# kritsanan1/Qwen3-TTS

Measured on AMD Instinct MI355X. Metric: audio-seconds/sec (RTF) + p50 first-packet latency, 1.7B @ batch 1/8, 1->8 GPU, higher is better.
Workload: dtype bf16; 1 GPU; Qwen3-TTS-12Hz-1.7b-customvoice B=8/GPU x 200-token prompts, streaming text, 256 frames + codec decode; global_batch=8, seq_len=200, frames=256, parallelism=dp1

## Files before the change

### include/qwen3tts_amd.h

```cpp
#ifndef QWEN3TTS_AMD_H
#define QWEN3TTS_AMD_H

#ifdef __cplusplus
extern "C" {
#endif

enum { QT_F32 = 0, QT_BF16 = 1 };
enum { QT_ACT_NONE = 0, QT_ACT_SILU = 1, QT_ACT_GELU = 2, QT_ACT_RELU = 3, QT_ACT_SIGMOID = 4,
       QT_ACT_RELU_TANH = 5  };
enum { QT_AACT_NONE = 0, QT_AACT_ELU = 1 };
enum { QT_PAD_ZERO = 0, QT_PAD_REFLECT = 1, QT_PAD_REPLICATE = 2 };
enum { QT_EPI_STORE = 0, QT_EPI_ADD = 1, QT_EPI_SWIGLU = 2 };
enum { QT_OK = 0, QT_ERR_ARG = -1, QT_ERR_SHAPE = -2, QT_ERR_DTYPE = -3, QT_ERR_LAUNCH = -4 };

const char* qt_build_id(void);

typedef struct qt_gemm_args {
  int M, N, K;
  int a_dtype, w_dtype, o_dtype;
  const void* A;
  long long lda;
  const int* a_index;
  const void* W;
  const float* gamma;
// ... 38 lines not shown
  const float* cos_tab; const float* sin_tab;
  const int* rope_pos; const int* row_batch; const int* kv_pos;
  float* q_out;
  void* k_cache; void* v_cache; int kv_dtype; int Lmax;
} qt_qkv_args;
int qt_qkv_post(const qt_qkv_args* args, void* stream);

typedef struct qt_attn_args {
  int R, Hq, Hkv, D, Lmax, window;
  const float* q;
  const void* k_cache; const void* v_cache; int kv_dtype;
  const int* row_batch; const int* row_start; const int* row_len;
  void* out; int o_dtype;
  int max_keys;
} qt_attn_args;
int qt_attention(const qt_attn_args* args, void* stream);

typedef struct qt_decode_attn_args {
  int R, Hq, Hkv, D, Lmax, window;
  const float* qkv;
  const float* q_norm; const float* k_norm; float eps;
  const float* cos_tab; const float* sin_tab;
  const int* rope_pos; const int* row_batch; const int* kv_pos; const int* row_start;
  void* k_cache; void* v_cache; int kv_dtype;
  void* out; int o_dtype;
  int const_pos;
  int nsplit;
  void* ws; long long ws_bytes;
} qt_decode_attn_args;
long long qt_decode_attn_ws_bytes(int R, int Hq, int Hkv, int D, int nsplit);
int qt_decode_attention(const qt_decode_attn_args* args, void* stream);
int qt_small_prefill_attention(const qt_decode_attn_args* args, int T, void* stream);

typedef struct qt_attn_oproj_args {
  int R, Hq, Hkv, D, Lmax;
  const float* qkv;
  const float* q_norm; const float* k_norm; float eps;
  const float* cos_tab; const float* sin_tab;
  const int* rope_pos; const int* kv_pos; const int* row_start; int const_pos;
  void* k_cache; void* v_cache; int kv_dtype;
  const void* w_o; int w_dtype; int N;
  float* x; long long ldx;
  void* x16; long long ldx16;
  void* ws; long long ws_bytes;
} qt_attn_oproj_args;
int qt_decode_attn_oproj(const qt_attn_oproj_args* args, void* stream);
long long qt_attn_oproj_ws_bytes(int N, int Hkv);
typedef struct qt_cp_step_args {
  int R, n_layers, Lmax, const_pos, V;
  float eps;
  const float* cos_tab; const float* sin_tab;
  const void* w_qkv[8]; const void* w_o[8]; const void* w_gu[8]; const void* w_down[8];
  const float* q_norm[8]; const float* k_norm[8];
  void* k_cache[8]; void* v_cache[8];
  const void* w_lm;
  const float* x; long long ldx;
  const float* qkv0; long long ldq;
  float* logits; long long ldl;
  void* ws; long long ws_bytes;
} qt_cp_step_args;
int qt_cp_step(const qt_cp_step_args* args, void* stream);
int qt_cp_prefill(const qt_cp_step_args* args, void* stream);
long long qt_cp_step_ws_bytes(void);
long long qt_cp_step_dbg_bytes(void);
int qt_cp_step_supported(int H, int I, int Hq, int Hkv, int D, int n_layers, int V);

int qt_attn_oproj_resident_blocks(void);

typedef struct qt_talker_tail_args {
  int R; float eps;
  const void* att; long long lda;
  float* x; long long ldx;
  const void* w_o; const void* w_gu; const void* w_down;
  const void* w_qkv_next;
  float* qkv; long long ldq;
  void* ws; long long ws_bytes;
  int H, I;
} qt_talker_tail_args;
int qt_talker_tail(const qt_talker_tail_args* args, void* stream);
long long qt_talker_tail_ws_bytes(void);
long long qt_talker_tail_stamp_bytes(void);
long long qt_talker_tail_dbg_bytes(void);
int qt_talker_tail_supported(int H, int I, int Hq, int D, int qkv_w);

typedef struct qt_sample_row {
  float temperature; float top_p; float rep_penalty; int top_k;
  int do_sample; int reserved; unsigned long long seed;
} qt_sample_row;

typedef struct qt_sample_args {
  const float* logits; int R; int V; long long ld;
  unsigned char* seen; float rep_penalty;
  const int* n_generated; int min_new_tokens; int eos_id;
  int suppress_lo, suppress_hi, suppress_keep; int ignore_eos;
  unsigned char* finished;
  int do_sample; int top_k; float top_p; float temperature;
  unsigned long long seed; const int* step; int substep;
  int* tok_out;
  int* codes; long long codes_ld; int codes_w; int codes_col; int codes_step_off;
  int row_base;
  const float* emb_table; int emb_dim; float* emb_out; long long emb_ld;
  const unsigned long long* seed_ptr;
  float debug_u;
  void* emb_out16; long long emb_ld16;
  const float* emb2_table; int emb2_dim; float* emb2_out; long long emb2_ld;
  int algo;
  int ctr_stride;
  const int* philox_row;
  const int* force; int* pick;
  const qt_sample_row* rows;
} qt_sample_args;
int qt_sample(const qt_sample_args* args, void* stream);
long long qt_sample_row_bytes(void);
long long qt_sample_args_bytes(void);
int qt_cp_step_sampled(const qt_cp_step_args* args, const qt_sample_args* sample, void* stream);

int qt_rmsnorm(const float* x, const float* gamma, float eps, float* out, int M, int N, void* stream);
int qt_rmsnorm_rec(const float* x, const float* gamma, float eps, float* out, int M, int N, float* rec,
                   long long rec_ld, const int* step, int step_off, int step_stride, void* stream);

int qt_gather_rows(const void* table, int dtype, const int* idx, int M, int H, float* out, long long ldo, void* stream);

int qt_frame_embed(const void* emb0, const void* emb_cp, int dtype, int V0, int Vcp, int G, int H,
                   const int* codes, long long codes_ld, const int* step, int step_stride, const float* trailing,
                   int T, const float* pad, float* x, void* x16, int B, void* stream);

int qt_advance(int* counters, int n, void* stream);
int qt_advance_rows(int* counters, int B, int nfields, int cap, void* stream);

int qt_trail_append(const float* rows, const int* slots, float* trailing, int B, int T, int H, int n, void* stream);

int qt_stream_window(void* hist, const void* x, void* xin, int dtype, int B, int H, int n, int C,
                     int rows_per_frame, int head, const int* rows, void* stream);
int qt_stream_rows(int* nf, const int* rows, int B, int n, int* pos, int* row_len, void* stream);

int qt_rvq_gather(const float* tables, int Q, int n_first, int cb_size, int dim, const int* codes, int B, int T,
                  float* out_first, float* out_rest, void* stream);
int qt_snake(const void* x, void* y, int dtype, long long rows, int C, const float* alpha, const float* inv_beta,
             void* stream);
int qt_dwconv_ln(const void* x, int dtype, int B, int T, int C, const float* w, const float* b, const float* ln_w,
                 const float* ln_b, float eps, void* out, void* stream);
int qt_clamp_pcm(const void* x, int dtype, long long n, float* out, void* stream);

enum { QT_PCM_F32 = 0, QT_PCM_S16 = 1 };
typedef struct qt_resample_row {
  const float* src;
  void* out;
  const float* hist_in;
  float* hist_out;
  long long pos;
  long long m0;
  int n, count, flush, reserved;
} qt_resample_row;
typedef struct qt_resample_args {
  int up, down, half, taps, H, format, B, reserved;
  const float* table;
  const qt_resample_row* rows;
} qt_resample_args;
int qt_resample(const qt_resample_args* a, void* stream);

int qt_pad_time(const void* x, long long ldx, const void* x2, long long ldx2, int dtype, int B, int T, int C, int left,
                int right, int mode, int t_total, void* out, long long ldo, void* stream);
int qt_zero_tail(void* x, int dtype, int B, int Tp, int v, int C, long long ldx, void* stream);
int qt_layernorm(const float* x, long long ldx, const float* w, const float* b, float eps, void* out, int o_dtype,
                 long long ldo, int M, int N, void* stream);
long long qt_rvq_encode_ws_bytes(int R, int D, int cb);
// ... 16 lines not shown
```

### qwen3-tts_amd/qwen_tts/_hip.py

```python
from __future__ import annotations

import ctypes
import os

import torch

HERE = os.path.dirname(os.path.abspath(__file__))
LIB_PATH = os.environ.get("QWEN3TTS_AMD_LIB",
                          os.path.join(os.path.dirname(HERE), "lib", "libqwen3tts_amd.so"))

F32, BF16 = 0, 1
ACT_NONE, ACT_SILU, ACT_GELU, ACT_RELU, ACT_SIGMOID, ACT_RELU_TANH = 0, 1, 2, 3, 4, 5
AACT_NONE, AACT_ELU = 0, 1
PAD_ZERO, PAD_REFLECT, PAD_REPLICATE = 0, 1, 2
EPI_STORE, EPI_ADD, EPI_SWIGLU = 0, 1, 2
ERRORS = {-1: "bad argument", -2: "bad shape", -3: "unsupported dtype", -4: "launch failed"}

c_int, c_ll, c_float, c_void_p, c_ull = ctypes.c_int, ctypes.c_longlong, ctypes.c_float, ctypes.c_void_p, ctypes.c_ulonglong


class GemmArgs(ctypes.Structure):
    _fields_ = [("M", c_int), ("N", c_int), ("K", c_int), ("a_dtype", c_int), ("w_dtype", c_int), ("o_dtype", c_int),
                ("A", c_void_p), ("lda", c_ll), ("a_index", c_void_p), ("W", c_void_p), ("gamma", c_void_p),
                ("eps", c_float), ("rmsnorm", c_int), ("bias", c_void_p), ("colscale", c_void_p), ("act", c_int), ("epi", c_int),
                ("out", c_void_p), ("ldo", c_ll), ("taps", c_int), ("dil", c_int), ("cin", c_int),
                ("cin_pad", c_int), ("t_in", c_int), ("t_out", c_int), ("t_off", c_int),
                ("ws", c_void_p), ("ws_bytes", c_ll), ("splitk", c_int),
                ("snake_alpha", c_void_p), ("snake_inv_beta", c_void_p), ("a_act", c_int),
                ("out2", c_void_p), ("ldo2", c_ll)]

GEMM_WS_MIN = 4 << 20

(ROUTE_NONE, ROUTE_IM2COL, ROUTE_GEMV, ROUTE_SK, ROUTE_CONV_N1, ROUTE_WT_1x8, ROUTE_WT_2x8, ROUTE_WT_4x4, ROUTE_PF2,
 ROUTE_PF, ROUTE_IGEMM) = range(11)
ROUTE_NAMES = ["NONE", "IM2COL", "GEMV", "SK", "CONV_N1", "WT_1x8", "WT_2x8", "WT_4x4", "PF2", "PF", "IGEMM"]


class GemmRouteInfo(ctypes.Structure):
    _fields_ = [(n, c_int) for n in ("route", "inner", "ks", "mr", "wpb", "u", "fold", "nt_loads", "pf2_cfg", "pf2_ks",
                                     "ntb", "mi", "sk_mi", "ws_split")]


class QkvArgs(ctypes.Structure):
    _fields_ = [("R", c_int), ("Hq", c_int), ("Hkv", c_int), ("D", c_int), ("qkv", c_void_p), ("q_norm", c_void_p),
                ("k_norm", c_void_p), ("eps", c_float), ("cos_tab", c_void_p), ("sin_tab", c_void_p),
                ("rope_pos", c_void_p), ("row_batch", c_void_p), ("kv_pos", c_void_p), ("q_out", c_void_p),
                ("k_cache", c_void_p), ("v_cache", c_void_p), ("kv_dtype", c_int), ("Lmax", c_int)]


class AttnArgs(ctypes.Structure):
    _fields_ = [("R", c_int), ("Hq", c_int), ("Hkv", c_int), ("D", c_int), ("Lmax", c_int), ("window", c_int),
                ("q", c_void_p), ("k_cache", c_void_p), ("v_cache", c_void_p), ("kv_dtype", c_int),
                ("row_batch", c_void_p), ("row_start", c_void_p), ("row_len", c_void_p), ("out", c_void_p),
                ("o_dtype", c_int), ("max_keys", c_int)]


class DecodeAttnArgs(ctypes.Structure):
    _fields_ = [("R", c_int), ("Hq", c_int), ("Hkv", c_int), ("D", c_int), ("Lmax", c_int), ("window", c_int),
                ("qkv", c_void_p), ("q_norm", c_void_p), ("k_norm", c_void_p), ("eps", c_float),
                ("cos_tab", c_void_p), ("sin_tab", c_void_p), ("rope_pos", c_void_p), ("row_batch", c_void_p),
                ("kv_pos", c_void_p), ("row_start", c_void_p), ("k_cache", c_void_p), ("v_cache", c_void_p),
                ("kv_dtype", c_int), ("out", c_void_p), ("o_dtype", c_int), ("const_pos", c_int), ("nsplit", c_int),
                ("ws", c_void_p), ("ws_bytes", c_ll)]


class AttnOprojArgs(ctypes.Structure):
    _fields_ = [("R", c_int), ("Hq", c_int), ("Hkv", c_int), ("D", c_int), ("Lmax", c_int), ("qkv", c_void_p),
                ("q_norm", c_void_p), ("k_norm", c_void_p), ("eps", c_float), ("cos_tab", c_void_p), ("sin_tab", c_void_p),
                ("rope_pos", c_void_p), ("kv_pos", c_void_p), ("row_start", c_void_p), ("const_pos", c_int),
                ("k_cache", c_void_p), ("v_cache", c_void_p), ("kv_dtype", c_int), ("w_o", c_void_p), ("w_dtype", c_int),
                ("N", c_int), ("x", c_void_p), ("ldx", c_ll), ("x16", c_void_p), ("ldx16", c_ll), ("ws", c_void_p),
                ("ws_bytes", c_ll)]


P8 = c_void_p * 8


class CpStepArgs(ctypes.Structure):
    _fields_ = [("R", c_int), ("n_layers", c_int), ("Lmax", c_int), ("const_pos", c_int), ("V", c_int),
                ("eps", c_float), ("cos_tab", c_void_p), ("sin_tab", c_void_p),
                ("w_qkv", P8), ("w_o", P8), ("w_gu", P8), ("w_down", P8), ("q_norm", P8), ("k_norm", P8),
                ("k_cache", P8), ("v_cache", P8), ("w_lm", c_void_p), ("x", c_void_p), ("ldx", c_ll),
                ("qkv0", c_void_p), ("ldq", c_ll), ("logits", c_void_p), ("ldl", c_ll), ("ws", c_void_p),
                ("ws_bytes", c_ll)]


class TalkerTailArgs(ctypes.Structure):
    _fields_ = [("R", c_int), ("eps", ctypes.c_float), ("att", c_void_p), ("lda", c_ll), ("x", c_void_p), ("ldx", c_ll),
                ("w_o", c_void_p), ("w_gu", c_void_p), ("w_down", c_void_p), ("w_qkv_next", c_void_p),
                ("qkv", c_void_p), ("ldq", c_ll), ("ws", c_void_p), ("ws_bytes", c_ll), ("H", c_int), ("I", c_int)]


class SampleRow(ctypes.Structure):
    _fields_ = [("temperature", c_float), ("top_p", c_float), ("rep_penalty", c_float), ("top_k", c_int),
                ("do_sample", c_int), ("reserved", c_int), ("seed", c_ull)]


class SampleArgs(ctypes.Structure):
    _fields_ = [("logits", c_void_p), ("R", c_int), ("V", c_int), ("ld", c_ll), ("seen", c_void_p),
                ("rep_penalty", c_float), ("n_generated", c_void_p), ("min_new_tokens", c_int), ("eos_id", c_int),
                ("suppress_lo", c_int), ("suppress_hi", c_int), ("suppress_keep", c_int), ("ignore_eos", c_int),
                ("finished", c_void_p), ("do_sample", c_int), ("top_k", c_int), ("top_p", c_float),
                ("temperature", c_float), ("seed", c_ull), ("step", c_void_p), ("substep", c_int),
                ("tok_out", c_void_p), ("codes", c_void_p), ("codes_ld", c_ll), ("codes_w", c_int),
                ("codes_col", c_int), ("codes_step_off", c_int), ("row_base", c_int),
                ("emb_table", c_void_p), ("emb_dim", c_int), ("emb_out", c_void_p), ("emb_ld", c_ll),
                ("seed_ptr", c_void_p), ("debug_u", c_float), ("emb_out16", c_void_p), ("emb_ld16", c_ll),
                ("emb2_table", c_void_p), ("emb2_dim", c_int), ("emb2_out", c_void_p), ("emb2_ld", c_ll),
                ("algo", c_int), ("ctr_stride", c_int), ("philox_row", c_void_p), ("force", c_void_p),
                ("pick", c_void_p), ("rows", c_void_p)]


PCM_F32, PCM_S16 = 0, 1


class ResampleRow(ctypes.Structure):
    _fields_ = [("src", c_void_p), ("out", c_void_p), ("hist_in", c_void_p), ("hist_out", c_void_p), ("pos", c_ll),
                ("m0", c_ll), ("n", c_int), ("count", c_int), ("flush", c_int), ("reserved", c_int)]


class ResampleArgs(ctypes.Structure):
    _fields_ = [("up", c_int), ("down", c_int), ("half", c_int), ("taps", c_int), ("H", c_int), ("format", c_int),
                ("B", c_int), ("reserved", c_int), ("table", c_void_p), ("rows", ctypes.POINTER(ResampleRow))]


EXPORTS = ["qt_gemm", "qt_gemm_route", "qt_tile_weight", "qt_qkv_post", "qt_attention", "qt_decode_attention", "qt_decode_attn_ws_bytes",
           "qt_rmsnorm_rec", "qt_small_prefill_attention",
           "qt_decode_attn_oproj", "qt_attn_oproj_ws_bytes", "qt_attn_oproj_resident_blocks",
           "qt_cp_step", "qt_cp_prefill", "qt_cp_step_sampled", "qt_cp_step_ws_bytes", "qt_cp_step_supported", "qt_cp_step_dbg_bytes",
           "qt_talker_tail", "qt_talker_tail_ws_bytes", "qt_talker_tail_stamp_bytes", "qt_talker_tail_dbg_bytes",
           "qt_talker_tail_supported",
           "qt_sample", "qt_sample_row_bytes", "qt_sample_args_bytes", "qt_rmsnorm", "qt_gather_rows", "qt_frame_embed", "qt_advance", "qt_advance_rows",
           "qt_stream_window", "qt_stream_rows", "qt_trail_append",
           "qt_rvq_gather", "qt_snake", "qt_dwconv_ln", "qt_clamp_pcm", "qt_resample",
           "qt_pad_time", "qt_zero_tail", "qt_layernorm", "qt_rvq_encode", "qt_rvq_encode_ws_bytes", "qt_mel_logmag", "qt_time_stats",
           "qt_scale_add", "qt_bcast_rows", "qt_build_id"]

_LIB = None
BUILD_ID = None


def source_digest(probe=False):
    bpath = os.path.join(os.path.dirname(HERE), "build.py")
    if not os.path.exists(bpath) or not os.path.isdir(os.path.join(os.path.dirname(HERE), "csrc")):
        return None
    import importlib.util
    spec = importlib.util.spec_from_file_location("_qt_build", bpath)
    mod = importlib.util.module_from_spec(spec)
    spec.loader.exec_module(mod)
    return mod.source_digest(probe=probe) + ("-probe" if probe else "")


def load_library(path: str = LIB_PATH):
    if not os.path.exists(path):
        raise RuntimeError(f"HIP library not found at {path}: run `python qwen3-tts_amd/build.py` "
                           "(or __graft_entry__.build()); there is no CPU fallback")
    L = ctypes.CDLL(path)
    L.qt_build_id.restype = ctypes.c_char_p
    L.qt_build_id.argtypes = []
    bid = L.qt_build_id().decode()
    want = source_digest(probe=os.path.basename(path).endswith("_probe.so")) if path == LIB_PATH else None
    if want is not None and bid != want and os.environ.get("QT_ALLOW_STALE_LIB") != "1":
        raise RuntimeError(f"{path} was built from other sources (build id {bid}, sources {want}): rebuild with "
                           "`python qwen3-tts_amd/build.py`")
    global BUILD_ID
    BUILD_ID = bid
    P = c_void_p
    sig = {
        "qt_gemm": [P, P], "qt_gemm_route": [P, P], "qt_tile_weight": [P, c_int, c_int, c_int, P, P], "qt_qkv_post": [P, P],
        "qt_attention": [P, P], "qt_decode_attention": [P, P], "qt_sample": [P, P],
        "qt_rmsnorm": [P, P, c_float, P, c_int, c_int, P],
        "qt_rmsnorm_rec": [P, P, c_float, P, c_int, c_int, P, c_ll, P, c_int, c_int, P],
        "qt_small_prefill_attention": [P, c_int, P],
        "qt_gather_rows": [P, c_int, P, c_int, c_int, P, c_ll, P],
        "qt_frame_embed": [P, P, c_int, c_int, c_int, c_int, c_int, P, c_ll, P, c_int, P, c_int, P, P, P, c_int, P],
        "qt_advance": [P, c_int, P],
        "qt_advance_rows": [P, c_int, c_int, c_int, P],
        "qt_trail_append": [P, P, P, c_int, c_int, c_int, c_int, P],
        "qt_stream_window": [P, P, P, c_int, c_int, c_int, c_int, c_int, c_int, c_int, P, P],
        "qt_stream_rows": [P, P, c_int, c_int, P, P, P],
        "qt_rvq_gather": [P, c_int, c_int, c_int, c_int, P, c_int, c_int, P, P, P],
        "qt_snake": [P, P, c_int, c_ll, c_int, P, P, P],
        "qt_dwconv_ln": [P, c_int, c_int, c_int, c_int, P, P, P, P, c_float, P, P],
        "qt_clamp_pcm": [P, c_int, c_ll, P, P],
        "qt_resample": [P, P],
        "qt_decode_attn_ws_bytes": [c_int, c_int, c_int, c_int, c_int],
        "qt_decode_attn_oproj": [P, P],
        "qt_attn_oproj_ws_bytes": [c_int, c_int],
        "qt_attn_oproj_resident_blocks": [],
        "qt_cp_step": [P, P], "qt_cp_prefill": [P, P], "qt_cp_step_sampled": [P, P, P], "qt_cp_step_ws_bytes": [], "qt_cp_step_dbg_bytes": [],
        "qt_cp_step_supported": [c_int, c_int, c_int, c_int, c_int, c_int, c_int],
        "qt_talker_tail": [P, P], "qt_talker_tail_ws_bytes": [], "qt_talker_tail_stamp_bytes": [], "qt_talker_tail_dbg_bytes": [],
        "qt_talker_tail_supported": [c_int, c_int, c_int, c_int, c_int],
        "qt_pad_time": [P, c_ll, P, c_ll, c_int, c_int, c_int, c_int, c_int, c_int, c_int, c_int, P, c_ll, P],
        "qt_zero_tail": [P, c_int, c_int, c_int, c_int, c_int, c_ll, P],
        "qt_layernorm": [P, c_ll, P, P, c_float, P, c_int, c_ll, c_int, c_int, P],
        "qt_rvq_encode": [P, c_ll, P, P, c_int, c_int, c_int, c_int, P, c_ll, P, c_ll, P],
        "qt_rvq_encode_ws_bytes": [c_int, c_int, c_int],
        "qt_mel_logmag": [P, c_ll, c_int, c_int, P, c_int, P, c_ll, P],
        "qt_time_stats": [P, c_int, c_ll, P, c_ll, c_int, c_int, c_int, c_float, P, P, c_ll, P],
        "qt_scale_add": [P, c_ll, P, c_ll, P, c_ll, c_int, c_int, c_int, c_int, P, c_ll, P],
        "qt_bcast_rows": [P, c_ll, c_int, c_int, c_int, P, c_int, c_ll, P],
        "qt_sample_row_bytes": [], "qt_sample_args_bytes": [],
    }
    for name, args in sig.items():
        f = getattr(L, name)
        f.argtypes = args
        f.restype = c_ll if name.endswith(("_ws_bytes", "_row_bytes", "_args_bytes")) else c_int
    return L


def lib():
    global _LIB
    if _LIB is None:
        if not torch.cuda.is_available():
            raise RuntimeError("qwen_tts (MI355X build) needs a ROCm GPU: no device visible and no CPU fallback")
        _LIB = load_library()
    return _LIB


def env_int(name: str, default: int) -> int:
    v = os.environ.get(name)
    if v is None:
        return default
    import re
    m = re.match(r"\s*([+-]?\d+)", v)
    return int(m.group(1)) if m else 0


PROBE = os.path.basename(LIB_PATH).endswith("_probe.so")


def lib_knob(name: str, default: int) -> int:
    return env_int(name, default) if PROBE else default


def check(rc: int, what: str):
    if rc != 0:
        raise RuntimeError(f"{what} failed: {ERRORS.get(rc, rc)}")


def ptr(t):
    return None if t is None else t.data_ptr()


def stream():
    return torch.cuda.current_stream().cuda_stream


def dtype_code(dt: torch.dtype) -> int:
    if dt == torch.float32:
        return F32
    if dt == torch.bfloat16:
        return BF16
    raise ValueError(f"unsupported dtype {dt}")
```

### qwen3-tts_amd/qwen_tts/codec.py

```python
from __future__ import annotations

import math
from typing import Dict, List

import torch

from . import _hip
from . import kernels as K


def _w(W, name, dev):
    t = W[name]
    if not isinstance(t, torch.Tensor):
        t = torch.from_numpy(t)
    return t.to(dev).float()


class CodecDecoder:
    def __init__(self, ccfg: dict, weights: Dict[str, torch.Tensor], dtype="bf16", device="cuda"):
        _hip.lib()
        self.ccfg = ccfg
        self.d = d = ccfg["decoder_config"]
        self.dev = dev = torch.device(device)
        self.wdt = wdt = torch.bfloat16 if dtype == "bf16" else torch.float32
        self.adt = wdt
        W = weights
        g = lambda n: _w(W, n, dev)
        Q = d["num_quantizers"]
        tabs = []
        for q in range(Q):
            grp, j = ("rvq_first", q) if q == 0 else ("rvq_rest", q - 1)
            p = f"decoder.quantizer.{grp}.vq.layers.{j}._codebook"
            tabs.append(g(f"{p}.embedding_sum") / g(f"{p}.cluster_usage").clamp(min=1e-5)[:, None])
        self.tables = torch.stack(tabs).contiguous()
        self.cb_dim = self.tables.shape[-1]
        self.proj_first = K.tile_linear(g("decoder.quantizer.rvq_first.output_proj.weight")[:, :, 0], wdt)
        self.proj_rest = K.tile_linear(g("decoder.quantizer.rvq_rest.output_proj.weight")[:, :, 0], wdt)
        self.pre_conv = K.tile_conv(g("decoder.pre_conv.conv.weight"), g("decoder.pre_conv.conv.bias"), wdt)
        pt = "decoder.pre_transformer"
        self.hid = d["hidden_size"]
        self.heads = d["num_attention_heads"]
        self.kvh = d["num_key_value_heads"]
        self.hd = self.hid // self.heads
        self.inp = K.tile_linear(g(f"{pt}.input_proj.weight"), wdt, g(f"{pt}.input_proj.bias"))
        self.outp = K.tile_linear(g(f"{pt}.output_proj.weight"), wdt, g(f"{pt}.output_proj.bias"), gamma=g(f"{pt}.norm.weight"))
        self.tnorm = g(f"{pt}.norm.weight").contiguous()
        self.layers = []
        for i in range(d["num_hidden_layers"]):
            p = f"{pt}.layers.{i}"
            self.layers.append(dict(
                qkv=K.tile_linear(torch.cat([g(f"{p}.self_attn.q_proj.weight"), g(f"{p}.self_attn.k_proj.weight"),
                                             g(f"{p}.self_attn.v_proj.weight")]), wdt, gamma=g(f"{p}.input_layernorm.weight")),
                o=K.tile_linear(g(f"{p}.self_attn.o_proj.weight"), wdt),
                gu=K.tile_swiglu(g(f"{p}.mlp.gate_proj.weight"), g(f"{p}.mlp.up_proj.weight"), wdt,
                                 gamma=g(f"{p}.post_attention_layernorm.weight")),
                down=K.tile_linear(g(f"{p}.mlp.down_proj.weight"), wdt),
                ln1=g(f"{p}.input_layernorm.weight").contiguous(), ln2=g(f"{p}.post_attention_layernorm.weight").contiguous(),
                ls1=g(f"{p}.self_attn_layer_scale.scale").contiguous(), ls2=g(f"{p}.mlp_layer_scale.scale").contiguous()))
        self.cos, self.sin = K.rope_tables(self.hd, d["rope_theta"], 512, dev)
        self.lat = d["latent_dim"]
        self.ups = []
        for i, f in enumerate(d["upsampling_ratios"]):
            p = f"decoder.upsample.{i}"
            self.ups.append(dict(
                f=f, tconv=K.tile_transconv(g(f"{p}.0.conv.weight"), g(f"{p}.0.conv.bias"), wdt, f),
                dw_w=g(f"{p}.1.dwconv.conv.weight")[:, 0, :].contiguous(), dw_b=g(f"{p}.1.dwconv.conv.bias"),
                ln_w=g(f"{p}.1.norm.weight"), ln_b=g(f"{p}.1.norm.bias"),
                pw1=K.tile_linear(g(f"{p}.1.pwconv1.weight"), wdt, g(f"{p}.1.pwconv1.bias")),
                pw2=K.tile_linear(g(f"{p}.1.pwconv2.weight"), wdt, g(f"{p}.1.pwconv2.bias")),
                gamma=g(f"{p}.1.gamma").contiguous()))
        self.conv0 = K.tile_conv(g("decoder.decoder.0.conv.weight"), g("decoder.decoder.0.conv.bias"), wdt)
        ds = d["decoder_dim"]
        self.blocks = []
        snake = lambda p: (torch.exp(g(f"{p}.alpha")).contiguous(),
                           (1.0 / (torch.exp(g(f"{p}.beta")) + 1e-9)).contiguous())
        for i, r in enumerate(d["upsample_rates"]):
            p = f"decoder.decoder.{i + 1}.block"
            units = []
            for j, dil in enumerate((1, 3, 9)):
                q = f"{p}.{j + 2}"
                units.append(dict(dil=dil, s1=snake(f"{q}.act1"), s2=snake(f"{q}.act2"),
                                  c1=K.tile_conv(g(f"{q}.conv1.conv.weight"), g(f"{q}.conv1.conv.bias"), wdt, dil),
                                  c2=K.tile_conv(g(f"{q}.conv2.conv.weight"), g(f"{q}.conv2.conv.bias"), wdt)))
            self.blocks.append(dict(r=r, cin=ds // 2 ** i, cout=ds // 2 ** (i + 1), s=snake(f"{p}.0"),
                                    tconv=K.tile_transconv(g(f"{p}.1.conv.weight"), g(f"{p}.1.conv.bias"), wdt, r),
                                    units=units))
        n = len(d["upsample_rates"])
        self.c_last = ds // 2 ** n
        self.s_last = snake(f"decoder.decoder.{n + 1}")
        self.conv_last = K.tile_conv(g(f"decoder.decoder.{n + 2}.conv.weight"), g(f"decoder.decoder.{n + 2}.conv.bias"),
                                     wdt)
        self.total_upsample = int(math.prod(d["upsample_rates"]) * math.prod(d["upsampling_ratios"]))
        self._slots = {}
        torch.cuda.synchronize()

    def _conv(self, x, Wt, B, t_in, t_out, t_off, out, cin, epi=_hip.EPI_STORE, act=_hip.ACT_NONE, snake=None):
        K.gemm(x, Wt, out, B * t_out, cin, Wt.N, conv=(t_in, t_out, t_off, getattr(Wt, "dil", 1)), epi=epi, act=act,
               snake=snake)

    def _causal(self, x, Wt, B, T, out, cin, epi=_hip.EPI_STORE, snake=None):
        dil = getattr(Wt, "dil", 1)
        self._conv(x, Wt, B, T, T, -(Wt.taps - 1) * dil, out, cin, epi, snake=snake)

    def _transformer(self, h, B, T):
        dev, R = self.dev, B * T
        hid, nh, nkv, D = self.hid, self.heads, self.kvh, self.hd
        x = torch.empty(R, self.inp.N, dtype=torch.float32, device=dev)
        K.gemm(h, self.inp, x, R, self.lat, self.inp.N)
        if self.cos.shape[0] < T:
            self.cos, self.sin = K.rope_tables(D, self.d["rope_theta"], T + 64, dev)
        pos = torch.arange(T, device=dev, dtype=torch.int32).repeat(B)
        meta_b = torch.arange(B, device=dev, dtype=torch.int32).repeat_interleave(T)
        row_len = pos + 1
        row_start = torch.zeros_like(pos)
        qkv_w = (nh + 2 * nkv) * D
        qkv = torch.empty(R, qkv_w, dtype=torch.float32, device=dev)
        q = torch.empty(R, nh * D, dtype=torch.float32, device=dev)
        att = torch.empty(R, nh * D, dtype=torch.float32, device=dev)
        hmid = torch.empty(R, self.d["intermediate_size"], dtype=torch.float32, device=dev)
        kc = torch.empty(B, nkv, T, D, dtype=torch.float32, device=dev)
        vc = torch.empty_like(kc)
        eps, win = self.d["rms_norm_eps"], self.d["sliding_window"]
        for L in self.layers:
            K.gemm(x, L["qkv"], qkv, R, hid, qkv_w, rms=True, eps=eps)
            K.qkv_post(qkv, R, nh, nkv, D, None, None, eps, self.cos, self.sin, pos, meta_b, pos, q, kc, vc, T)
            K.attention(q, R, nh, nkv, D, kc, vc, T, meta_b, row_start, row_len, att, min(win, T), window=win)
            K.gemm(att, L["o"], x, R, nh * D, hid, colscale=L["ls1"], epi=_hip.EPI_ADD)
            K.gemm(x, L["gu"], hmid, R, hid, self.d["intermediate_size"], rms=True, eps=eps, epi=_hip.EPI_SWIGLU)
            K.gemm(hmid, L["down"], x, R, self.d["intermediate_size"], hid, colscale=L["ls2"], epi=_hip.EPI_ADD)
        y = torch.empty(R, self.lat, dtype=self.adt, device=dev)
        K.gemm(x, self.outp, y, R, hid, self.lat, rms=True, eps=eps)
        return y

    def forward(self, codes: torch.Tensor) -> torch.Tensor:
        B, T, Qn = codes.shape
        dev, adt = self.dev, self.adt
        codes = codes.to(dev, torch.int32).contiguous()
        o1 = torch.empty(B * T, self.cb_dim, dtype=torch.float32, device=dev)
        o2 = torch.empty_like(o1)
        K.rvq_gather(self.tables, Qn, 1, self.tables.shape[1], self.cb_dim, codes, B, T, o1, o2)
        cd = self.proj_first.N
        h = torch.empty(B * T, cd, dtype=adt, device=dev)
        K.gemm(o1, self.proj_first, h, B * T, self.cb_dim, cd)
        K.gemm(o2, self.proj_rest, h, B * T, self.cb_dim, cd, epi=_hip.EPI_ADD)
        x = torch.empty(B * T, self.pre_conv.N, dtype=adt, device=dev)
        self._causal(h, self.pre_conv, B, T, x, cd)
        x = self._transformer(x, B, T)
        L = T
        C = self.lat
        for u in self.ups:
            f = u["f"]
            y = torch.empty(B * L * f, C, dtype=adt, device=dev)
            self._conv(x, u["tconv"], B, L, L, 0, y, C)
            L *= f
            z = torch.empty_like(y)
            K.dwconv_ln(y, B, L, C, u["dw_w"], u["dw_b"], u["ln_w"], u["ln_b"], 1e-6, z)
            hmid = torch.empty(B * L, u["pw1"].N, dtype=adt, device=dev)
            K.gemm(z, u["pw1"], hmid, B * L, C, u["pw1"].N, act=_hip.ACT_GELU)
            K.gemm(hmid, u["pw2"], y, B * L, u["pw1"].N, C, colscale=u["gamma"], epi=_hip.EPI_ADD)
            x = y
        ds = self.d["decoder_dim"]
        y = torch.empty(B * L, self.conv0.N, dtype=adt, device=dev)
        self._causal(x, self.conv0, B, L, y, C)
        x, C = y, ds
        for blk in self.blocks:
            r, cout = blk["r"], blk["cout"]
            Lo = (L - 1) * r
            y = torch.empty(B * Lo, cout, dtype=adt, device=dev)
            self._conv(x, blk["tconv"], B, L, L - 1, 0, y, C, snake=blk["s"])
            L, C, x = Lo, cout, y
            bb = torch.empty_like(x)
            for un in blk["units"]:
                self._causal(x, un["c1"], B, L, bb, C, snake=un["s1"])
                self._causal(bb, un["c2"], B, L, x, C, epi=_hip.EPI_ADD, snake=un["s2"])
        out = torch.empty(B * L, self.conv_last.N, dtype=torch.float32, device=dev)
        self._conv(x, self.conv_last, B, L, L, -(self.conv_last.taps - 1), out, C, snake=self.s_last)
        pcm = out[:, 0].contiguous()
        K.clamp_pcm(pcm, pcm.numel(), pcm)
        return pcm.view(B, L)

    def stream(self, B: int, max_frames: int) -> "CodecStream":
        return CodecStream(self, B, max_frames)

    def row_stream(self, B: int, max_frames: int, n_max: int = 8) -> "RowCodecStream":
        return RowCodecStream(self, B, max_frames, n_max)

    def _acquire_slot(self, B, max_frames) -> "_StreamSlot":
        pool = self._slots.setdefault((B, max_frames), [])
        for sl in pool:
            if not sl.busy:
                sl.reset()
                sl.busy = True
                return sl
        sl = _StreamSlot(self, B, max_frames)
        sl.busy = True
        pool.append(sl)
        return sl

    def chunked_decode(self, codes: torch.Tensor, chunk_size=300, left_context_size=25) -> torch.Tensor:
        wavs, start, T = [], 0, codes.shape[1]
        while start < T:
            end = min(start + chunk_size, T)
            ctx = left_context_size if start - left_context_size > 0 else start
            w = self.forward(codes[:, start - ctx:end])
            wavs.append(w[:, ctx * self.total_upsample:])
            start = end
        return torch.cat(wavs, -1)

    def decode(self, audio_codes: torch.Tensor) -> List[torch.Tensor]:
        cb = self.tables.shape[1]
        if audio_codes.numel() and (int(audio_codes.min()) < 0 or int(audio_codes.max()) >= cb):
            raise ValueError(f"audio codes must lie in [0, {cb}); got [{int(audio_codes.min())}, "
                             f"{int(audio_codes.max())}]")
        if audio_codes.shape[1] == 0:
            return [torch.zeros(0, device=self.dev) for _ in range(audio_codes.shape[0])]
        wav = self.chunked_decode(audio_codes)
        lengths = (audio_codes[..., 0] > 0).sum(1) * self.ccfg["decode_upsample_rate"]
        return [a[:int(l)] for a, l in zip(wav, lengths)]


class _StreamSlot:

    def __init__(self, dec: "CodecDecoder", B: int, max_frames: int):
        dev = dec.dev
        self.kc = [torch.zeros(B, dec.kvh, max_frames, dec.hd, dtype=torch.float32, device=dev) for _ in dec.layers]
        self.vc = [torch.zeros_like(k) for k in self.kc]
        self.nf_dev = torch.zeros(1, dtype=torch.int32, device=dev)
        self.hist = {}
        self.graphs = {}
        self.uses = {}
        self.busy = False
        self.ws = K.new_workspace(dev)

    def reset(self):
        for h in self.hist.values():
            h.zero_()
        self.nf_dev.zero_()


CODEC_GRAPH = _hip.lib_knob("QT_CODEC_GRAPH", 1) != 0


class CodecStream:

    def __init__(self, dec: "CodecDecoder", B: int, max_frames: int):
        self.dec, self.B, self.max_frames = dec, B, max_frames
        d = dec.d
        if dec.cos.shape[0] < max_frames:
            dec._old_rope = getattr(dec, "_old_rope", []) + [(dec.cos, dec.sin)]
            dec.cos, dec.sin = K.rope_tables(dec.hd, d["rope_theta"], max_frames + 64, dec.dev)
        self.slot = dec._acquire_slot(B, max_frames)
        self.nf = 0
        self.pcm = torch.zeros(B, dec.total_upsample * max_frames, dtype=torch.float32, device=dec.dev)
        self.ns = 0

# ... 346 lines not shown
```

### qwen3-tts_amd/qwen_tts/kernels.py

```python
from __future__ import annotations

import contextlib
import ctypes
import gc
import threading
from dataclasses import dataclass
from typing import Optional

import torch
import torch.nn.functional as F

from . import _hip
from ._hip import ptr, stream, check

KT_OF = {torch.bfloat16: 32, torch.float32: 16}


@dataclass
class Tiled:
    w: torch.Tensor
    N: int
    Np: int
    K: int
    Kp: int
# ... 223 lines not shown
    a.nsplit = nsplit
    if ws is not None:
        a.ws, a.ws_bytes = ptr(ws), ws.numel() * ws.element_size()
    check(_hip.lib().qt_decode_attention(ctypes.byref(a), stream()), "qt_decode_attention")


def attn_oproj_ws_bytes(N, Hkv):
    return int(_hip.lib().qt_attn_oproj_ws_bytes(N, Hkv))


def decode_attn_oproj(qkv, R, Hq, Hkv, D, q_norm, k_norm, eps, cos, sin, kc, vc, Lmax, w_o: "Tiled", x, *,
                      const_pos=-1, rope_pos=None, kv_pos=None, row_start=None, x16=None, ws=None):
    a = _hip.AttnOprojArgs()
    a.R, a.Hq, a.Hkv, a.D, a.Lmax = R, Hq, Hkv, D, Lmax
    a.qkv, a.q_norm, a.k_norm, a.eps = ptr(qkv), ptr(q_norm), ptr(k_norm), eps
    a.cos_tab, a.sin_tab = ptr(cos), ptr(sin)
    a.rope_pos, a.kv_pos, a.row_start, a.const_pos = ptr(rope_pos), ptr(kv_pos), ptr(row_start), const_pos
    a.k_cache, a.v_cache, a.kv_dtype = ptr(kc), ptr(vc), _hip.dtype_code(kc.dtype)
    a.w_o, a.w_dtype, a.N = ptr(w_o.w), _hip.dtype_code(w_o.dtype), w_o.N
    a.x, a.ldx = ptr(x), x.stride(0)
    if x16 is not None:
        a.x16, a.ldx16 = ptr(x16), x16.stride(0)
    if ws is not None:
        a.ws, a.ws_bytes = ptr(ws), ws.numel() * ws.element_size()
    check(_hip.lib().qt_decode_attn_oproj(ctypes.byref(a), stream()), "qt_decode_attn_oproj")


def cp_step_ws_bytes():
    return int(_hip.lib().qt_cp_step_ws_bytes())


def cp_step_supported(H, I, Hq, Hkv, D, n_layers, V) -> bool:
    return bool(_hip.lib().qt_cp_step_supported(H, I, Hq, Hkv, D, n_layers, V))


def _cp_args(layers, w_lm: "Tiled", x, R, kcs, vcs, Lmax, const_pos, cos, sin, eps, logits, ws):
    a = _hip.CpStepArgs()
    a.R, a.n_layers, a.Lmax, a.const_pos, a.V, a.eps = R, len(layers), Lmax, const_pos, w_lm.N, eps
    a.cos_tab, a.sin_tab = ptr(cos), ptr(sin)
    for i, L in enumerate(layers):
        a.w_qkv[i], a.w_o[i], a.w_gu[i], a.w_down[i] = ptr(L.qkv.w), ptr(L.o.w), ptr(L.gu.w), ptr(L.down.w)
        a.q_norm[i], a.k_norm[i] = ptr(L.q_norm), ptr(L.k_norm)
        a.k_cache[i], a.v_cache[i] = ptr(kcs[i]), ptr(vcs[i])
    a.w_lm = ptr(w_lm.w)
    a.x, a.ldx = ptr(x), x.stride(0)
    a.logits, a.ldl = ptr(logits), logits.stride(0)
    a.ws, a.ws_bytes = ptr(ws), ws.numel() * ws.element_size()
    return a


def cp_step(layers, w_lm: "Tiled", x, qkv0, R, kcs, vcs, Lmax, const_pos, cos, sin, eps, logits, ws, sample=None):
    a = _cp_args(layers, w_lm, x, R, kcs, vcs, Lmax, const_pos, cos, sin, eps, logits, ws)
    a.qkv0, a.ldq = ptr(qkv0), qkv0.stride(0)
    if sample is not None:
        check(_hip.lib().qt_cp_step_sampled(ctypes.byref(a), ctypes.byref(sample), stream()), "qt_cp_step_sampled")
        return
    check(_hip.lib().qt_cp_step(ctypes.byref(a), stream()), "qt_cp_step")


def cp_prefill(layers, w_lm: "Tiled", x, R, kcs, vcs, Lmax, cos, sin, eps, logits, ws):
    a = _cp_args(layers, w_lm, x, R, kcs, vcs, Lmax, 0, cos, sin, eps, logits, ws)
    check(_hip.lib().qt_cp_prefill(ctypes.byref(a), stream()), "qt_cp_prefill")


def talker_tail_ws_bytes():
    return int(_hip.lib().qt_talker_tail_ws_bytes())


def talker_tail_supported(H, I, Hq, D, qkv_w) -> bool:
    return bool(_hip.lib().qt_talker_tail_supported(H, I, Hq, D, qkv_w))


def talker_tail(att, x, R, layer, next_layer, qkv, eps, ws):
    a = _hip.TalkerTailArgs()
    a.R, a.eps = R, eps
    a.att, a.lda = ptr(att), att.stride(0)
    a.x, a.ldx = ptr(x), x.stride(0)
    a.w_o, a.w_gu, a.w_down = ptr(layer.o.w), ptr(layer.gu.w), ptr(layer.down.w)
    a.w_qkv_next = ptr(next_layer.qkv.w) if next_layer is not None else None
    a.qkv, a.ldq = (ptr(qkv), qkv.stride(0)) if next_layer is not None else (None, 0)
    a.ws, a.ws_bytes = ptr(ws), ws.numel() * ws.element_size()
    a.H, a.I = layer.o.N, layer.gu.N // 2
    check(_hip.lib().qt_talker_tail(ctypes.byref(a), stream()), "qt_talker_tail")


def sample(logits, R, V, ld, tok_out, *, seen=None, rep_penalty=1.0, n_generated=None, min_new_tokens=0, eos_id=-1,
           suppress=(0, 0, -1), ignore_eos=False, finished=None, do_sample=False, top_k=0, top_p=1.0,
           temperature=1.0, seed=0, step=None, substep=0, codes=None, codes_ld=0, codes_w=16, codes_col=0,
           codes_step_off=0, row_base=0, emb=None, seed_ptr=None, debug_u=-1.0, emb16=None, emb2=None, algo=0,
           ctr_stride=0, philox_row=None, force=None, pick=None, rows=None, launch=True):
    a = _hip.SampleArgs()
    a.logits, a.R, a.V, a.ld = ptr(logits), R, V, ld
    a.seen, a.rep_penalty = ptr(seen), rep_penalty
    a.n_generated, a.min_new_tokens, a.eos_id = ptr(n_generated), min_new_tokens, eos_id
    a.suppress_lo, a.suppress_hi, a.suppress_keep = suppress
    a.ignore_eos, a.finished = int(ignore_eos), ptr(finished)
    a.do_sample, a.top_k, a.top_p, a.temperature = int(do_sample), int(top_k or 0), float(top_p), float(temperature)
    a.seed, a.step, a.substep, a.tok_out = seed & (2 ** 64 - 1), ptr(step), substep, ptr(tok_out)
    a.codes, a.codes_ld, a.codes_w, a.codes_col, a.codes_step_off = ptr(codes), codes_ld, codes_w, codes_col, codes_step_off
    a.row_base = row_base
    a.seed_ptr, a.debug_u, a.algo = ptr(seed_ptr), float(debug_u), int(algo)
    a.ctr_stride, a.philox_row = int(ctr_stride), ptr(philox_row)
    a.force, a.pick = ptr(force), ptr(pick)
    if rows is not None:
        assert rows.dtype == torch.uint8 and rows.is_contiguous() and rows.shape[0] >= R and rows.shape[1] == ROW_BYTES
        a.rows = ptr(rows)
    if emb is not None:
        a.emb_table, a.emb_dim, a.emb_out, a.emb_ld = ptr(emb[0]), emb[0].shape[1], ptr(emb[1]), emb[2]
        if emb16 is not None:
            a.emb_out16, a.emb_ld16 = ptr(emb16[0]), emb16[1]
        if emb2 is not None:
            a.emb2_table, a.emb2_dim, a.emb2_out, a.emb2_ld = ptr(emb2[0]), emb2[0].shape[1], ptr(emb2[1]), emb2[2]
    if not launch:
        return a
    check(_hip.lib().qt_sample(ctypes.byref(a), stream()), "qt_sample")


ROW_BYTES = ctypes.sizeof(_hip.SampleRow)


def sample_rows_table(n, device):
    return torch.zeros(n, ROW_BYTES, dtype=torch.uint8, device=device)


def pack_sample_rows(records):
    arr = (_hip.SampleRow * len(records))()
    for rec, (do_sample, top_k, top_p, temperature, rep_penalty, seed) in zip(arr, records):
        rec.temperature, rec.top_p, rec.rep_penalty = float(temperature), float(top_p), float(rep_penalty)
        rec.top_k, rec.do_sample, rec.seed = int(top_k or 0), int(bool(do_sample)), int(seed) & (2 ** 64 - 1)
    host = torch.empty(len(records), ROW_BYTES, dtype=torch.uint8, pin_memory=True)
    ctypes.memmove(host.data_ptr(), ctypes.addressof(arr), len(records) * ROW_BYTES)
    return host


def upload_sample_rows(table, b0, records):
    table[b0:b0 + len(records)].copy_(pack_sample_rows(records), non_blocking=True)


def rmsnorm(x, g, eps, out, M, N, rec=None, step=None, step_off=0, step_stride=0):
    if rec is None:
        check(_hip.lib().qt_rmsnorm(ptr(x), ptr(g), eps, ptr(out), M, N, stream()), "qt_rmsnorm")
    else:
        check(_hip.lib().qt_rmsnorm_rec(ptr(x), ptr(g), eps, ptr(out), M, N, ptr(rec), rec.stride(0), ptr(step),
                                        step_off, step_stride, stream()), "qt_rmsnorm_rec")


def gather_rows(table, idx, M, H, out, ldo):
    check(_hip.lib().qt_gather_rows(ptr(table), _hip.dtype_code(table.dtype), ptr(idx), M, H, ptr(out), ldo, stream()),
          "qt_gather_rows")


def frame_embed(e0, ecp, G, H, codes, codes_ld, step, trailing, T, pad, x, B, x16=None, step_stride=0):
    check(_hip.lib().qt_frame_embed(ptr(e0), ptr(ecp), _hip.dtype_code(e0.dtype), e0.shape[0], ecp.shape[1], G, H,
                                    ptr(codes), codes_ld, ptr(step), step_stride, ptr(trailing), T, ptr(pad), ptr(x),
                                    ptr(x16), B,
                                    stream()),
          "qt_frame_embed")


def advance(counters, n):
    check(_hip.lib().qt_advance(ptr(counters), n, stream()), "qt_advance")


def advance_rows(counters, B, nfields, cap):
    check(_hip.lib().qt_advance_rows(ptr(counters), B, nfields, cap, stream()), "qt_advance_rows")

# ... 92 lines not shown
```

Before: 246.4 audio-seconds/sec.

## Fuse codec residual unit (snake, k7 conv, snake, k1 conv, residual) into one kernel

```diff
diff --git a/include/qwen3tts_amd.h b/include/qwen3tts_amd.h
--- a/include/qwen3tts_amd.h
+++ b/include/qwen3tts_amd.h
@@ -144,6 +144,16 @@
 long long qt_talker_tail_stamp_bytes(void);
 long long qt_talker_tail_dbg_bytes(void);
 int qt_talker_tail_supported(int H, int I, int Hq, int D, int qkv_w);
+
+typedef struct qt_codec_resunit_args {
+  int B, L, C, dil;
+  int a_dtype, w_dtype;
+  const void* x_in; void* x_out;
+  const void* w1; const float* b1; const float* s1_alpha; const float* s1_inv_beta;
+  const void* w2; const float* b2; const float* s2_alpha; const float* s2_inv_beta;
+} qt_codec_resunit_args;
+int qt_codec_resunit(const qt_codec_resunit_args* args, void* stream);
+int qt_codec_resunit_supported(const qt_codec_resunit_args* args);
 
 typedef struct qt_sample_row {
   float temperature; float top_p; float rep_penalty; int top_k;
diff --git a/qwen3-tts_amd/csrc/codec_unit.hip b/qwen3-tts_amd/csrc/codec_unit.hip
--- /dev/null
+++ b/qwen3-tts_amd/csrc/codec_unit.hip
@@ -0,0 +1,233 @@
+#include "common.h"
+
+namespace {
+
+constexpr int CU_TAPS = 7;
+constexpr int CU_MAX_DIL = 9;
+
+constexpr int unit_wpe(int C, int MI) { return C == 96 ? (MI == 4 ? 2 : 4) : (MI == 1 ? 3 : 2); }
+
+template <int C, int MI>
+__global__ __launch_bounds__(256) __attribute__((amdgpu_waves_per_eu(unit_wpe(C, MI)))) void codec_unit_k(
+    qt_codec_resunit_args p) {
+  constexpr int BM = 64 * MI;
+  constexpr int RT = BM / 32;
+  constexpr int NCH = C / 32;
+  constexpr int CT = C / 32;
+  constexpr int G = C / 8;
+  constexpr int LDW = C + 8;
+  constexpr int RPI = 256 / G;
+  constexpr int NR = BM * G / 256;
+  static_assert(BM * G % 256 == 0, "output tile groups divide over the block");
+  extern __shared__ __attribute__((aligned(16))) unsigned char cu_smem[];
+  bf16_t* img = (bf16_t*)cu_smem;
+  const int tid = threadIdx.x, lane = tid & 63, w = tid >> 6;
+  const int lm = lane & 15, lk = lane >> 4;
+  const int dil = p.dil, halo = (CU_TAPS - 1) * dil, WR = BM + halo;
+  const int tiles_t = (p.L + BM - 1) / BM;
+  const int bi = blockIdx.x / tiles_t, t0 = (blockIdx.x - bi * tiles_t) * BM;
+  const bf16_t* xin = (const bf16_t*)p.x_in + (long long)bi * p.L * C;
+  bf16_t* xout = (bf16_t*)p.x_out + (long long)bi * p.L * C;
+
+  {
+    const int g = tid % G, r0 = tid / G;
+    if (r0 < RPI) {
+      float sa[8], sib[8];
+      load8f(p.s1_alpha + g * 8, sa);
+      load8f(p.s1_inv_beta + g * 8, sib);
+      for (int rb = r0; rb < WR; rb += 4 * RPI) {
+        u32x4_t raw[4];
+#pragma unroll
+        for (int u = 0; u < 4; ++u) {
+          const int r = rb + u * RPI, ti = t0 - halo + r;
+          raw[u] = u32x4_t{0u, 0u, 0u, 0u};
+          if (r < WR && ti >= 0 && ti < p.L) raw[u] = *(const u32x4_t*)(xin + (long long)ti * C + g * 8);
+        }
+#pragma unroll
+        for (int u = 0; u < 4; ++u) {
+          const int r = rb + u * RPI;
+          if (r >= WR) break;
+          float v[8];
+#pragma unroll
+          for (int i = 0; i < 4; ++i) {
+            v[2 * i] = __uint_as_float(raw[u][i] << 16);
+            v[2 * i + 1] = __uint_as_float(raw[u][i] & 0xFFFF0000u);
+          }
+#pragma unroll
+          for (int e = 0; e < 8; ++e) {
+            const float sn = __sinf(v[e] * sa[e]);
+            v[e] = v[e] + sib[e] * (sn * sn);
+          }
+          *(u32x4_t*)(img + r * LDW + g * 8) =
+              u32x4_t{pack2bf(v[0], v[1]), pack2bf(v[2], v[3]), pack2bf(v[4], v[5]), pack2bf(v[6], v[7])};
+        }
+      }
+    }
+  }
+
+  const int wrow = (w >> 1) * (BM / 2);
+  const int nt0 = (w & 1) * CT;
+  f32x4_t acc[RT][CT];
+#pragma unroll
+  for (int i = 0; i < RT; ++i)
+#pragma unroll
+    for (int q = 0; q < CT; ++q) acc[i][q] = f32x4_t{0.f, 0.f, 0.f, 0.f};
+
+  {
+    constexpr int KT = CU_TAPS * NCH;
+    const bf16_t* Wb = (const bf16_t*)p.w1 + lane * 8;
+    u32x4_t cur[CT], nxt[CT];
+#pragma unroll
+    for (int q = 0; q < CT; ++q) cur[q] = *(const u32x4_t*)(Wb + ((size_t)(nt0 + q) * KT) * 512);
+    __syncthreads();
+#pragma unroll 1
+    for (int c = 0; c < NCH; ++c) {
+      const bf16_t* wa = img + (wrow + lm) * LDW + c * 32 + lk * 8;
+#pragma unroll
+      for (int j = 0; j < CU_TAPS; ++j) {
+        const int kn = j + 1 < CU_TAPS ? (j + 1) * NCH + c : (c + 1 < NCH ? c + 1 : c);
+#pragma unroll
+        for (int q = 0; q < CT; ++q) nxt[q] = *(const u32x4_t*)(Wb + ((size_t)(nt0 + q) * KT + kn) * 512);
+        u32x4_t af[RT];
+#pragma unroll
+        for (int i = 0; i < RT; ++i) af[i] = *(const u32x4_t*)(wa + (i * 16 + j * dil) * LDW);
+#pragma unroll
+        for (int i = 0; i < RT; ++i)
+#pragma unroll
+          for (int q = 0; q < CT; ++q)
+            acc[i][q] = __builtin_amdgcn_mfma_f32_16x16x32_bf16(__builtin_bit_cast(bf16x8_t, af[i]),
+                                                                __builtin_bit_cast(bf16x8_t, cur[q]), acc[i][q], 0, 0, 0);
+#pragma unroll
+        for (int q = 0; q < CT; ++q) cur[q] = nxt[q];
+      }
+    }
+  }
+  __syncthreads();
+
+  u32x4_t xr[NR];
+#pragma unroll
+  for (int u = 0; u < NR; ++u) {
+    const int q = tid + u * 256, r = q / G, g = q - r * G;
+    xr[u] = u32x4_t{0u, 0u, 0u, 0u};
+    if (t0 + r < p.L) xr[u] = *(const u32x4_t*)(xin + (long long)(t0 + r) * C + g * 8);
+  }
+
+#pragma unroll
+  for (int q = 0; q < CT; ++q) {
+    const int n = (nt0 + q) * 16 + lm;
+    const float b1 = p.b1 ? p.b1[n] : 0.f, a2 = p.s2_alpha[n], ib2 = p.s2_inv_beta[n];
+#pragma unroll
+    for (int i = 0; i < RT; ++i)
+#pragma unroll
+      for (int e = 0; e < 4; ++e) {
+        const float h = bf2f(f2bf(acc[i][q][e] + b1));
+        const float sn = __sinf(h * a2);
+        img[(wrow + i * 16 + lk * 4 + e) * LDW + n] = f2bf(h + ib2 * (sn * sn));
+        acc[i][q][e] = 0.f;
+      }
+  }
+
+  {
+    const bf16_t* Wb = (const bf16_t*)p.w2 + lane * 8;
+    u32x4_t cur[CT], nxt[CT];
+#pragma unroll
+    for (int q = 0; q < CT; ++q) cur[q] = *(const u32x4_t*)(Wb + ((size_t)(nt0 + q) * NCH) * 512);
+    __syncthreads();
+    const bf16_t* wa = img + (wrow + lm) * LDW + lk * 8;
+#pragma unroll
+    for (int c = 0; c < NCH; ++c) {
+      const int kn = c + 1 < NCH ? c + 1 : c;
+#pragma unroll
+      for (int q = 0; q < CT; ++q) nxt[q] = *(const u32x4_t*)(Wb + ((size_t)(nt0 + q) * NCH + kn) * 512);
+      u32x4_t af[RT];
+#pragma unroll
+      for (int i = 0; i < RT; ++i) af[i] = *(const u32x4_t*)(wa + i * 16 * LDW + c * 32);
+#pragma unroll
+      for (int i = 0; i < RT; ++i)
+#pragma unroll
+        for (int q = 0; q < CT; ++q)
+          acc[i][q] = __builtin_amdgcn_mfma_f32_16x16x32_bf16(__builtin_bit_cast(bf16x8_t, af[i]),
+                                                              __builtin_bit_cast(bf16x8_t, cur[q]), acc[i][q], 0, 0, 0);
+#pragma unroll
+      for (int q = 0; q < CT; ++q) cur[q] = nxt[q];
+    }
+  }
+  __syncthreads();
+
+#pragma unroll
+  for (int u = 0; u < NR; ++u) {
+    const int q = tid + u * 256, r = q / G, g = q - r * G;
+    *(u32x4_t*)(img + r * LDW + g * 8) = xr[u];
+  }
+  __syncthreads();
+#pragma unroll
+  for (int q = 0; q < CT; ++q) {
+    const int n = (nt0 + q) * 16 + lm;
+    const float b2 = p.b2 ? p.b2[n] : 0.f;
+#pragma unroll
+    for (int i = 0; i < RT; ++i)
+#pragma unroll
+      for (int e = 0; e < 4; ++e) {
+        bf16_t* s = img + (wrow + i * 16 + lk * 4 + e) * LDW + n;
+        *s = f2bf(bf2f(*s) + (acc[i][q][e] + b2));
+      }
+  }
+  __syncthreads();
+
+#pragma unroll
+  for (int u = 0; u < NR; ++u) {
+    const int q = tid + u * 256, r = q / G, g = q - r * G;
+    if (t0 + r < p.L) *(u32x4_t*)(xout + (long long)(t0 + r) * C + g * 8) = *(const u32x4_t*)(img + r * LDW + g * 8);
+  }
+}
+
+size_t unit_smem(int C, int bm, int dil) { return (size_t)(bm + (CU_TAPS - 1) * dil) * (C + 8) * sizeof(bf16_t); }
+
+template <int C, int MI>
+int launch_unit(const qt_codec_resunit_args& a, hipStream_t s) {
+  constexpr int BM = 64 * MI;
+  const size_t smem = unit_smem(C, BM, a.dil);
+  if (smem > (64u << 10) &&
+      hipFuncSetAttribute((const void*)codec_unit_k<C, MI>, hipFuncAttributeMaxDynamicSharedMemorySize,
+                          (int)unit_smem(C, BM, CU_MAX_DIL)) != hipSuccess)
+    return QT_ERR_LAUNCH;
+  const long long blocks = (long long)a.B * ((a.L + BM - 1) / BM);
+  hipLaunchKernelGGL((codec_unit_k<C, MI>), dim3((unsigned)blocks), dim3(256), smem, s, a);
+  return hipGetLastError() == hipSuccess ? QT_OK : QT_ERR_LAUNCH;
+}
+
+}
+
+static int unit_check(const qt_codec_resunit_args* a) {
+  if (!a) return QT_ERR_ARG;
+  if (a->a_dtype != QT_BF16 || a->w_dtype != QT_BF16) return QT_ERR_DTYPE;
+  if (a->C != 96 && a->C != 192) return QT_ERR_SHAPE;
+  if (a->dil != 1 && a->dil != 3 && a->dil != CU_MAX_DIL) return QT_ERR_SHAPE;
+  if (a->B < 1 || a->L < 1 || (long long)a->B * ((a->L + 63) / 64) > 0x7FFFFFFFLL) return QT_ERR_SHAPE;
+  if (!a->x_in || !a->x_out || !a->w1 || !a->w2 || !a->s1_alpha || !a->s1_inv_beta || !a->s2_alpha || !a->s2_inv_beta)
+    return QT_ERR_ARG;
+  if ((reinterpret_cast<uintptr_t>(a->x_in) | reinterpret_cast<uintptr_t>(a->x_out) | reinterpret_cast<uintptr_t>(a->w1) |
+       reinterpret_cast<uintptr_t>(a->w2) | reinterpret_cast<uintptr_t>(a->s1_alpha) |
+       reinterpret_cast<uintptr_t>(a->s1_inv_beta)) & 15)
+    return QT_ERR_ARG;
+  const unsigned long long bytes = (unsigned long long)a->B * a->L * a->C * sizeof(bf16_t);
+  const uintptr_t xi = reinterpret_cast<uintptr_t>(a->x_in), xo = reinterpret_cast<uintptr_t>(a->x_out);
+  if (xi < xo + bytes && xo < xi + bytes) return QT_ERR_ARG;
+  return QT_OK;
+}
+
+extern "C" int qt_codec_resunit_supported(const qt_codec_resunit_args* a) { return unit_check(a) == QT_OK; }
+
+extern "C" int qt_codec_resunit(const qt_codec_resunit_args* a, void* stream) {
+  const int rc = unit_check(a);
+  if (rc != QT_OK) return rc;
+  hipStream_t s = (hipStream_t)stream;
+  if constexpr (kProbe) {
+    const int mi = qt_knob("QT_CU_MI", 0);
+    if (a->C == 96 && mi == 1) return launch_unit<96, 1>(*a, s);
+    if (a->C == 96 && mi == 4) return launch_unit<96, 4>(*a, s);
+    if (a->C == 192 && (mi == 2 || mi == 4)) return launch_unit<192, 2>(*a, s);
+  }
+  if (a->C == 96) return launch_unit<96, 2>(*a, s);
+  return launch_unit<192, 1>(*a, s);
+}
diff --git a/qwen3-tts_amd/qwen_tts/_hip.py b/qwen3-tts_amd/qwen_tts/_hip.py
--- a/qwen3-tts_amd/qwen_tts/_hip.py
+++ b/qwen3-tts_amd/qwen_tts/_hip.py
@@ -89,6 +89,13 @@
     _fields_ = [("R", c_int), ("eps", ctypes.c_float), ("att", c_void_p), ("lda", c_ll), ("x", c_void_p), ("ldx", c_ll),
                 ("w_o", c_void_p), ("w_gu", c_void_p), ("w_down", c_void_p), ("w_qkv_next", c_void_p),
                 ("qkv", c_void_p), ("ldq", c_ll), ("ws", c_void_p), ("ws_bytes", c_ll), ("H", c_int), ("I", c_int)]
+
+
+class CodecResunitArgs(ctypes.Structure):
+    _fields_ = [("B", c_int), ("L", c_int), ("C", c_int), ("dil", c_int), ("a_dtype", c_int), ("w_dtype", c_int),
+                ("x_in", c_void_p), ("x_out", c_void_p),
+                ("w1", c_void_p), ("b1", c_void_p), ("s1_alpha", c_void_p), ("s1_inv_beta", c_void_p),
+                ("w2", c_void_p), ("b2", c_void_p), ("s2_alpha", c_void_p), ("s2_inv_beta", c_void_p)]
 
 
 class SampleRow(ctypes.Structure):
@@ -129,7 +136,7 @@
            "qt_decode_attn_oproj", "qt_attn_oproj_ws_bytes", "qt_attn_oproj_resident_blocks",
            "qt_cp_step", "qt_cp_prefill", "qt_cp_step_sampled", "qt_cp_step_ws_bytes", "qt_cp_step_supported", "qt_cp_step_dbg_bytes",
            "qt_talker_tail", "qt_talker_tail_ws_bytes", "qt_talker_tail_stamp_bytes", "qt_talker_tail_dbg_bytes",
-           "qt_talker_tail_supported",
+           "qt_talker_tail_supported", "qt_codec_resunit", "qt_codec_resunit_supported",
            "qt_sample", "qt_sample_row_bytes", "qt_sample_args_bytes", "qt_rmsnorm", "qt_gather_rows", "qt_frame_embed", "qt_advance", "qt_advance_rows",
            "qt_stream_window", "qt_stream_rows", "qt_trail_append",
            "qt_rvq_gather", "qt_snake", "qt_dwconv_ln", "qt_clamp_pcm", "qt_resample",
@@ -192,6 +199,7 @@
         "qt_cp_step_supported": [c_int, c_int, c_int, c_int, c_int, c_int, c_int],
         "qt_talker_tail": [P, P], "qt_talker_tail_ws_bytes": [], "qt_talker_tail_stamp_bytes": [], "qt_talker_tail_dbg_bytes": [],
         "qt_talker_tail_supported": [c_int, c_int, c_int, c_int, c_int],
+        "qt_codec_resunit": [P, P], "qt_codec_resunit_supported": [P],
         "qt_pad_time": [P, c_ll, P, c_ll, c_int, c_int, c_int, c_int, c_int, c_int, c_int, c_int, P, c_ll, P],
         "qt_zero_tail": [P, c_int, c_int, c_int, c_int, c_int, c_ll, P],
         "qt_layernorm": [P, c_ll, P, P, c_float, P, c_int, c_ll, c_int, c_int, P],
diff --git a/qwen3-tts_amd/qwen_tts/codec.py b/qwen3-tts_amd/qwen_tts/codec.py
--- a/qwen3-tts_amd/qwen_tts/codec.py
+++ b/qwen3-tts_amd/qwen_tts/codec.py
@@ -17,9 +17,11 @@
 
 
 class CodecDecoder:
-    def __init__(self, ccfg: dict, weights: Dict[str, torch.Tensor], dtype="bf16", device="cuda"):
+    def __init__(self, ccfg: dict, weights: Dict[str, torch.Tensor], dtype="bf16", device="cuda", fuse_units=True):
         _hip.lib()
         self.ccfg = ccfg
+        self.fuse_units = fuse_units
+        self._unit_fused = {}
         self.d = d = ccfg["decoder_config"]
         self.dev = dev = torch.device(device)
         self.wdt = wdt = torch.bfloat16 if dtype == "bf16" else torch.float32
@@ -102,6 +104,21 @@
         dil = getattr(Wt, "dil", 1)
         self._conv(x, Wt, B, T, T, -(Wt.taps - 1) * dil, out, cin, epi, snake=snake)
 
+    def _fuses(self, un, x, bb, B, L, C) -> bool:
+        if not self.fuse_units or self.adt != torch.bfloat16:
+            return False
+        key = (C, un["dil"], B, L, K.active_workspace(self.dev) is not None)
+        hit = self._unit_fused.get(key)
+        if hit is None:
+            hit = K.codec_resunit_supported(x, bb, B, L, C, un["c1"], un["s1"], un["c2"], un["s2"])
+            if hit:
+                c1 = un["c1"]
+                info = K.gemm_route(x, c1, bb, B * L, C, c1.N, conv=(L, L, -(c1.taps - 1) * un["dil"], un["dil"]),
+                                    snake=un["s1"])
+                hit = info.route == _hip.ROUTE_IGEMM
+            self._unit_fused[key] = hit
+        return hit
+
     def _transformer(self, h, B, T):
         dev, R = self.dev, B * T
         hid, nh, nkv, D = self.hid, self.heads, self.kvh, self.hd
@@ -171,6 +188,10 @@
             L, C, x = Lo, cout, y
             bb = torch.empty_like(x)
             for un in blk["units"]:
+                if self._fuses(un, x, bb, B, L, C):
+                    K.codec_resunit(x, bb, B, L, C, un["c1"], un["s1"], un["c2"], un["s2"])
+                    x, bb = bb, x
+                    continue
                 self._causal(x, un["c1"], B, L, bb, C, snake=un["s1"])
                 self._causal(bb, un["c2"], B, L, x, C, epi=_hip.EPI_ADD, snake=un["s2"])
         out = torch.empty(B * L, self.conv_last.N, dtype=torch.float32, device=dev)
diff --git a/qwen3-tts_amd/qwen_tts/kernels.py b/qwen3-tts_amd/qwen_tts/kernels.py
--- a/qwen3-tts_amd/qwen_tts/kernels.py
+++ b/qwen3-tts_amd/qwen_tts/kernels.py
@@ -329,6 +329,35 @@
     a.ws, a.ws_bytes = ptr(ws), ws.numel() * ws.element_size()
     a.H, a.I = layer.o.N, layer.gu.N // 2
     check(_hip.lib().qt_talker_tail(ctypes.byref(a), stream()), "qt_talker_tail")
+
+
+def _codec_resunit_args(x_in, x_out, B, L, C, c1: Tiled, s1, c2: Tiled, s2, dil=None):
+    a = _hip.CodecResunitArgs()
+    a.B, a.L, a.C, a.dil = B, L, C, getattr(c1, "dil", 1) if dil is None else dil
+    a.a_dtype, a.w_dtype = _hip.dtype_code(x_in.dtype), _hip.dtype_code(c1.dtype)
+    a.x_in, a.x_out = ptr(x_in), ptr(x_out)
+    a.w1, a.b1, a.s1_alpha, a.s1_inv_beta = ptr(c1.w), ptr(c1.bias), ptr(s1[0]), ptr(s1[1])
+    a.w2, a.b2, a.s2_alpha, a.s2_inv_beta = ptr(c2.w), ptr(c2.bias), ptr(s2[0]), ptr(s2[1])
+    return a
+
+
+def _is_resunit(C, c1: Tiled, c2: Tiled) -> bool:
+    return (c1.taps, c1.cin, c1.cin_pad, c1.N, c2.taps, c2.cin, c2.cin_pad, c2.N) == (7, C, C, C, 1, C, C, C) \
+        and c2.dtype == c1.dtype
+
+
+def codec_resunit_supported(x_in, x_out, B, L, C, c1: Tiled, s1, c2: Tiled, s2, dil=None) -> bool:
+    if not _is_resunit(C, c1, c2) or x_out.dtype != x_in.dtype:
+        return False
+    a = _codec_resunit_args(x_in, x_out, B, L, C, c1, s1, c2, s2, dil)
+    return bool(_hip.lib().qt_codec_resunit_supported(ctypes.byref(a)))
+
+
+def codec_resunit(x_in, x_out, B, L, C, c1: Tiled, s1, c2: Tiled, s2, dil=None):
+    if not _is_resunit(C, c1, c2) or x_out.dtype != x_in.dtype:
+        raise ValueError("codec_resunit: c1 / c2 are not a C -> C residual unit's k = 7 and k = 1 convs")
+    a = _codec_resunit_args(x_in, x_out, B, L, C, c1, s1, c2, s2, dil)
+    check(_hip.lib().qt_codec_resunit(ctypes.byref(a), stream()), "qt_codec_resunit")
 
 
 def sample(logits, R, V, ld, tok_out, *, seen=None, rep_penalty=1.0, n_generated=None, min_new_tokens=0, eos_id=-1,
```

New measurement: 250.0 audio-seconds/sec, median of 6. 1.5% higher.
